# JaneliaSciComp/BigStitcher-Spark

Measured on AMD Instinct MI355X. Metric: tile-pairs/sec phase-correlated (512^3 uint16), higher is better.
Workload: dtype f32+i64; 1 GPU; BASELINE.json configs[1]: 64x512^3 uint16 tile-pairs per GPU, ~10% x-overlap content, ds=1,1,1, peaks=5, subpixel, 8 distinct scenes, no collectives; pairs_per_gpu=64, tile=512^3, parallelism=dp1 hash-sharded pairs

## Files before the change

bigstitcher_spark_amd/csrc/bigstitch.hip:

```cpp

#include "../../include/bigstitch.h"

#include <hip/hip_runtime.h>

#include "rtest_walk.h"
#include "xfft_r4.h"

#include <chrono>
#include <climits>
#include <cmath>
#include <cstdio>
#include <cstdlib>
#include <cstring>
#include <condition_variable>
#include <functional>
#include <map>
#include <mutex>
#include <thread>
#include <string>
#include <vector>
#include <algorithm>

#define LPB_X 4
#define TPL_X 64
#define LPB_S 8
#define TPL_S 64

typedef unsigned long long u64;

struct f2 { float x, y; };

__device__ __forceinline__ f2 cmul(f2 a, f2 b) {
  return {a.x * b.x - a.y * b.y, a.x * b.y + a.y * b.x};
}
__device__ __forceinline__ f2 conjmul(f2 a, f2 b) {
  return {a.x * b.x + a.y * b.y, a.x * b.y - a.y * b.x};
}
__device__ __forceinline__ unsigned brev_n(unsigned j, int log2n) {
  return __brev(j) >> (32 - log2n);
}

template <int ES, int TPL>
__device__ __forceinline__ void fft_lds(f2 *data, long base, int n,
                                        int log2n, int tl, const f2 *tw,
                                        int dir) {
#define D_(e) data[base + (long)(e) * ES]
  int h = 1;
  if (log2n & 1) {
    for (int bf = tl; bf < (n >> 1); bf += TPL) {
      f2 u = D_(2 * bf), v = D_(2 * bf + 1);
      D_(2 * bf) = {u.x + v.x, u.y + v.y};
      D_(2 * bf + 1) = {u.x - v.x, u.y - v.y};
    }
    h = 2;
    __syncthreads();
  }
  for (; h < n; h <<= 2) {
    const int q = n >> 2;
    const int s1 = n / (2 * h), s2 = n / (4 * h);
    for (int g = tl; g < q; g += TPL) {
      int off = g % h, blk = g / h;
      int i = blk * 4 * h + off;
      f2 a = D_(i), b = D_(i + h), c = D_(i + 2 * h), d = D_(i + 3 * h);
      f2 w1 = tw[off * s1];
      if (dir < 0) w1.y = -w1.y;
      f2 t1 = cmul(b, w1), t2 = cmul(d, w1);
      f2 A = {a.x + t1.x, a.y + t1.y}, B = {a.x - t1.x, a.y - t1.y};
      f2 Cc = {c.x + t2.x, c.y + t2.y}, Dd = {c.x - t2.x, c.y - t2.y};
      f2 w2a = tw[off * s2], w2b = tw[(off + h) * s2];
      if (dir < 0) {
        w2a.y = -w2a.y;
        w2b.y = -w2b.y;
      }
      f2 u1 = cmul(Cc, w2a), u2 = cmul(Dd, w2b);
      D_(i) = {A.x + u1.x, A.y + u1.y};
      D_(i + 2 * h) = {A.x - u1.x, A.y - u1.y};
      D_(i + h) = {B.x + u2.x, B.y + u2.y};
      D_(i + 3 * h) = {B.x - u2.x, B.y - u2.y};
    }
    __syncthreads();
  }
#undef D_
}

template <int ES, int TPL>
__device__ __forceinline__ int fft_stockham(f2 *bufA, f2 *bufB, long base,
                                            int n, unsigned long long
                                                        factors,
                                            int tl, const f2 *tw,
// ... 1103 lines not shown
  for (unsigned lid = blockIdx.x * XW_WPB + wv; lid < nlines;
       lid += gridDim.x * XW_WPB) {
    const int z = (int)(lid / (unsigned)in.my);
    const int y = (int)(lid - (unsigned)z * (unsigned)in.my);
    const unsigned short *src =
        in.ptr + (in.oz + z) * in.sxy + (in.oy + y) * in.sx + in.ox;
    f2 v[E];
    if (((size_t)src & 3) == 0 && in.mx >= 2 * h) {
#pragma unroll
      for (int e = 0; e < E; ++e) {
        const unsigned w = ((const unsigned *)src)[lane + 64 * e];
        v[e] = {(float)(w & 0xFFFF), (float)(w >> 16)};
      }
    } else {
#pragma unroll
      for (int e = 0; e < E; ++e) {
        const int j = lane + 64 * e;
        v[e] = {2 * j < in.mx ? (float)src[2 * j] : 0.0f,
                2 * j + 1 < in.mx ? (float)src[2 * j + 1] : 0.0f};
      }
    }
    xf_wave_fft<E, +1>(v, tws, buf, lane);
    xf_wave_sync();
#pragma unroll
    for (int e = 0; e < E; ++e) buf[lane + 64 * e] = v[e];
    xf_wave_sync();
    f2 *o = out + ((long)z * py + y) * cxp;
#pragma unroll
    for (int e = 0; e < E; ++e) {
      const int k = lane + 64 * e;
      const f2 zm = buf[xf_mirror<E>(k)];
      if (k == 0) {
        f2 x0, xh;
        xf_unpack0(v[0], x0, xh);
        o[0] = x0;
        o[h] = xh;
      } else {
        o[k] = xf_unpack(v[e], zm, twu[e]);
      }
    }
  }
}

template <int E>
__global__ __launch_bounds__(64 * XW_WPB) void k_fft_x_inv_r4(
    const f2 *in, float *out, float *rowmax, long cxp, long nlines,
    const f2 *twg, const int *rows, const int *nrows_dev, int store_pcm,
    int store_rowmax) {
  constexpr int h = 64 * E;
  __shared__ f2 xb[XW_WPB][h];
  const int lane = threadIdx.x & 63;
  const int wv = __builtin_amdgcn_readfirstlane(threadIdx.x >> 6);
  f2 *buf = xb[wv];
  xf_twset<E, f2> tws;
  xf_load_tw<E>(tws, twg, lane, -1);
  f2 twp[E];
#pragma unroll
  for (int e = 0; e < E; ++e) twp[e] = twg[lane + 64 * e];
  if (rows) nlines = *nrows_dev;
  for (long li = (long)blockIdx.x * XW_WPB + wv; li < nlines;
       li += (long)gridDim.x * XW_WPB) {
    const long lid = rows ? (long)rows[li] : li;
    const f2 *src = in + lid * cxp;
    f2 v[E];
#pragma unroll
    for (int e = 0; e < E; ++e) {
      const int k = lane + 64 * e;
      v[e] = xf_prep(src[k], src[h - k], twp[e]);
    }
    xf_wave_fft<E, -1>(v, tws, buf, lane);
    if (store_pcm) {
      f2 *o = (f2 *)(out + lid * 2 * h);
#pragma unroll
      for (int e = 0; e < E; ++e)
        o[e * 64 + lane] = v[e];
    }
    if (store_rowmax) {
      float m = fmaxf(v[0].x, v[0].y);
#pragma unroll
      for (int e = 1; e < E; ++e) m = fmaxf(m, fmaxf(v[e].x, v[e].y));
      m = wave_max_f32(m);
      if (lane == 0) rowmax[lid] = m;
    }
  }
}


struct bs_peak {
  float v;
  int pad;
  long long idx;
};

__device__ __forceinline__ bool pk_better(float v, long long i, float v2,
                                          long long i2) {
  return (v > v2) || (v == v2 && i < i2);
}

__device__ void pk_insert(float (&tv)[5], long long (&ti)[5], float v,
                          long long i) {
  if (!pk_better(v, i, tv[4], ti[4])) return;
  tv[4] = v; ti[4] = i;
  for (int k = 4; k > 0 && pk_better(tv[k], ti[k], tv[k - 1], ti[k - 1]);
       --k) {
    float fv = tv[k]; tv[k] = tv[k - 1]; tv[k - 1] = fv;
    long long fi = ti[k]; ti[k] = ti[k - 1]; ti[k - 1] = fi;
  }
}

__device__ void pk_merge_shfl(float (&tv)[5], long long (&ti)[5]) {
  for (int off = 32; off >= 1; off >>= 1) {
    float ov[5]; long long oi[5];
    for (int k = 0; k < 5; ++k) {
      ov[k] = __shfl_down(tv[k], off);
      oi[k] = __shfl_down(ti[k], off);
    }
    for (int k = 0; k < 5; ++k) pk_insert(tv, ti, ov[k], oi[k]);
  }
}

struct pk_raw {
  float4 r[3];
  float el[3], er[3];
};

struct pk_win {
  float4 nm[3];
  float4 raw1;
  float4 cm1;
};

__device__ __forceinline__ pk_win pk_compute(const pk_raw &p, int lane,
                                             int nlt) {
  pk_win o;
#pragma unroll
  for (int k = 0; k < 3; ++k) {
    const float4 r = p.r[k];
    float lw = __shfl_up(r.w, 1);
    float rw = __shfl_down(r.x, 1);
    if (lane == 0) lw = p.el[k];
    if (lane == nlt - 1) rw = p.er[k];
    o.nm[k].x = fmaxf(fmaxf(lw, r.x), r.y);
    o.nm[k].y = fmaxf(fmaxf(r.x, r.y), r.z);
    o.nm[k].z = fmaxf(fmaxf(r.y, r.z), r.w);
    o.nm[k].w = fmaxf(fmaxf(r.z, r.w), rw);
    if (k == 1) {
      o.raw1 = r;
      o.cm1 = {fmaxf(lw, r.y), fmaxf(r.x, r.z), fmaxf(r.y, r.w),
               fmaxf(r.z, rw)};
    }
  }
  return o;
}

__device__ __forceinline__ float4 f4max(float4 a, float4 b) {
  return {fmaxf(a.x, b.x), fmaxf(a.y, b.y), fmaxf(a.z, b.z),
          fmaxf(a.w, b.w)};
}

#define PKW_CZ 64

template <bool UNUSED>
__device__ __forceinline__ void pk_body(const float *pcm, int px, int py,
                                        int pz, bs_peak *wgbuf) {
  __shared__ float wvs[4][5];
  __shared__ long long wis[4][5];
// ... 949 lines not shown
      std::lock_guard<std::mutex> lk(mu);
      stop = true;
    }
    cv.notify_all();
    for (auto &t : th) t.join();
  }
};

struct bs_slot {
  hipStream_t stream = nullptr;
  hipEvent_t peaks_ready = nullptr, done = nullptr;
  f2 *spec = nullptr;
  size_t spec_cap = 0;
  float *pcm = nullptr;
  size_t pcm_cap = 0;
  unsigned short *regbuf[2] = {nullptr, nullptr};
  size_t reg_cap[2] = {0, 0};
  bs_peak *wgpk = nullptr;
  size_t wgpk_cap = 0;
  bs_peak *dmerge = nullptr;
  bs_peak *dtop5 = nullptr;
  float *rowmax = nullptr;
  size_t rowmax_cap = 0;
  int *rowstamp = nullptr;
  size_t rowstamp_cap = 0;
  int *rowlist = nullptr;
  int row_epoch = 0;
  int pcm_sparse = 0;
  int row_listed = 0;
  f2 *twx = nullptr;
  int xinv_r4 = 0;
  int pk_prefilter = 0;
  bs_cand *dcands = nullptr;
  u64 *dsums = nullptr;
  long long *dpkidx = nullptr;
  float *dsubpix = nullptr;
  bs_peak *htop5 = nullptr;
  u64 *hsums = nullptr;
  float *hsubpix = nullptr;
  int Px = 0, Py = 0, Pz = 0, Cx = 0;
  long Cxp = 0;
  bs_region reg[2];
  int m[2][3];
  int dsf[3];
  std::vector<bs_hostcand> hc;
  long long pkidx_h[8];
  int npk = 0;
  size_t out_idx = 0;
  int stage = 0;
};

#define BS_NSLOTS 4

struct bs_ctx {
  int dev;
  int nslots = 2;
  std::map<int, f2 *> twiddles_full;
  hipStream_t stream;
  hipStream_t copy_stream = nullptr;
  bs_pool cpool;
  std::string err;
  std::map<int32_t, bs_view_rec> views;
  std::map<int, f2 *> twiddles;
  bs_slot slot[BS_NSLOTS];
  unsigned long long *synth_acc = nullptr;
  size_t synth_cap = 0;
  void *fuse_out = nullptr;
  size_t fuse_cap = 0;
  bs_dev_view *dviews = nullptr;
  size_t dviews_cap = 0;
  int *dvidx = nullptr;
  size_t dvidx_cap = 0;
  float *dblobs = nullptr;
  size_t dblobs_cap = 0;
  void *hstage[2] = {nullptr, nullptr};
  void *dvol_arena = nullptr;
  size_t dvol_cap = 0;
  hipEvent_t stage_ev[2] = {nullptr, nullptr};
  int peak_full = 0;
  int pcm_rows = 1;
  bs_slot *dbg_slot = nullptr;
  int corr_wide = 1;
  int xfft_fwd_r4 = 1, xfft_inv_r4 = 1;
  float *dbg_pcm = nullptr;
  bs_peak dbg_top5[5] = {};
  long dbg_px = 0, dbg_py = 0, dbg_pz = 0;
  float *dog_box = nullptr, *dog_g1 = nullptr, *dog_g2 = nullptr,
        *dog_d = nullptr;
  size_t dog_box_cap = 0, dog_g1_cap = 0, dog_g2_cap = 0, dog_d_cap = 0;
  long long *dog_cand = nullptr;
  size_t dog_cand_cap = 0;
  struct bs_dog_pt *dog_pts = nullptr;
  size_t dog_pts_cap = 0;
  unsigned int *dog_cnt = nullptr;
  size_t dog_cnt_cap = 0;
  size_t dog_init_cap = 65536;
  void *ip_buf[12] = {};
  size_t ip_cap[12] = {};
  int ip_split = 0;
  void *int_buf[8] = {};
  size_t int_cap[8] = {};
  bs_batch_stats stats{};
  std::vector<bs_ev> evs;
  std::vector<std::pair<hipEvent_t, hipEvent_t>> evpool;
  size_t evused = 0;
  std::mutex mu;
};

#define CHK(ctx, call)                                                      \
  do {                                                                      \
    hipError_t e_ = (call);                                                 \
    if (e_ != hipSuccess) {                                                 \
      (ctx)->err = std::string(#call) + ": " + hipGetErrorString(e_);       \
      return BS_EHIP;                                                       \
    }                                                                       \
  } while (0)

static thread_local std::string g_err;

extern "C" const char *bs_last_error(const bs_ctx *ctx) {
  return ctx ? ctx->err.c_str() : g_err.c_str();
}

static size_t rtest_alloc_bytes(size_t bytes) {
  return (bytes + 15) & ~(size_t)15;
}

static int ensure_dev(bs_ctx *c, void **p, size_t *cap, size_t need) {
  if (need <= *cap) return BS_OK;
  if (*p) (void)hipFree(*p);
  *p = nullptr;
  *cap = 0;
  hipError_t e = hipMalloc(p, need);
  if (e != hipSuccess) {
    c->err = std::string("hipMalloc: ") + hipGetErrorString(e);
    return BS_ENOMEM;
  }
  *cap = need;
  return BS_OK;
}

extern "C" int bs_ctx_create(bs_ctx **out, int device_id) {
  if (!out) return BS_EINVAL;
  int n = 0;
  if (hipGetDeviceCount(&n) != hipSuccess || device_id >= n) {
    g_err = "no HIP device (libbigstitch requires a GPU; the product path "
            "has no CPU fallback)";
    return BS_ENODEV;
  }
  bs_ctx *c = new bs_ctx();
  c->dev = device_id;
  if (const char *e = getenv("BS_SLOTS")) {
    int v = atoi(e);
    if (v >= 1 && v <= BS_NSLOTS) c->nslots = v;
  }
  if (const char *e = getenv("BS_PEAK_MODE"))
    c->peak_full = strcmp(e, "full") == 0;
  if (const char *e = getenv("BS_PCM_MODE"))
    c->pcm_rows = strcmp(e, "full") != 0;
  if (c->peak_full) c->pcm_rows = 0;
  if (const char *e = getenv("BS_CORR_MODE"))
    c->corr_wide = strcmp(e, "legacy") != 0;
  if (const char *e = getenv("BS_XFFT_MODE")) {
    c->xfft_fwd_r4 = strcmp(e, "r4") == 0 || strcmp(e, "r4fwd") == 0;
    c->xfft_inv_r4 = strcmp(e, "r4") == 0 || strcmp(e, "r4inv") == 0;
  }
  if (const char *e = getenv("BS_DOG_INIT_CAP")) {
    long v = atol(e);
    if (v >= 1) c->dog_init_cap = (size_t)v;
  }
  if (const char *e = getenv("BS_IP_SPLIT")) {
    int v = atoi(e);
    if (v >= 1) c->ip_split = v;
  }
  if (hipSetDevice(device_id) != hipSuccess ||
      hipStreamCreate(&c->stream) != hipSuccess ||
      hipStreamCreate(&c->copy_stream) != hipSuccess) {
    delete c;
    g_err = "hip init failed";
    return BS_ENODEV;
  }
  (void)hipFuncSetAttribute((const void *)k_fft_pass,
                            hipFuncAttributeMaxDynamicSharedMemorySize,
                            160 * 1024);
  (void)hipFuncSetAttribute((const void *)k_fft_pass_m,
                            hipFuncAttributeMaxDynamicSharedMemorySize,
                            160 * 1024);
  (void)hipFuncSetAttribute((const void *)k_fft_x_fwd_m,
                            hipFuncAttributeMaxDynamicSharedMemorySize,
                            160 * 1024);
  (void)hipFuncSetAttribute((const void *)k_fft_x_inv_m,
                            hipFuncAttributeMaxDynamicSharedMemorySize,
                            160 * 1024);
  (void)hipFuncSetAttribute((const void *)k_fft_pass_glds<2>,
                            hipFuncAttributeMaxDynamicSharedMemorySize,
                            160 * 1024);
  (void)hipFuncSetAttribute((const void *)k_fft_pass_glds<4>,
                            hipFuncAttributeMaxDynamicSharedMemorySize,
                            160 * 1024);
  (void)hipFuncSetAttribute((const void *)k_fft_pass_glds<8>,
                            hipFuncAttributeMaxDynamicSharedMemorySize,
                            160 * 1024);
  (void)hipFuncSetAttribute((const void *)k_fft_z_fused<1>,
                            hipFuncAttributeMaxDynamicSharedMemorySize,
                            160 * 1024);
  (void)hipFuncSetAttribute((const void *)k_fft_z_fused<2>,
                            hipFuncAttributeMaxDynamicSharedMemorySize,
                            160 * 1024);
  (void)hipFuncSetAttribute((const void *)k_fft_z_fused<4>,
                            hipFuncAttributeMaxDynamicSharedMemorySize,
                            160 * 1024);
  (void)hipFuncSetAttribute((const void *)k_fft_z_fused<8>,
                            hipFuncAttributeMaxDynamicSharedMemorySize,
                            160 * 1024);
  (void)hipFuncSetAttribute((const void *)k_fft_x_fwd,
                            hipFuncAttributeMaxDynamicSharedMemorySize,
                            64 * 1024);
  (void)hipFuncSetAttribute((const void *)k_fft_x_inv,
                            hipFuncAttributeMaxDynamicSharedMemorySize,
                            64 * 1024);
  bool ok = true;
  for (int s = 0; s < BS_NSLOTS; ++s) {
    bs_slot &sl = c->slot[s];
    ok = ok && hipStreamCreate(&sl.stream) == hipSuccess &&
         hipEventCreateWithFlags(&sl.peaks_ready, hipEventDisableTiming) ==
             hipSuccess &&
         hipEventCreateWithFlags(&sl.done, hipEventDisableTiming) ==
             hipSuccess &&
         hipMalloc(&sl.dmerge, 64 * 5 * sizeof(bs_peak)) == hipSuccess &&
         hipMalloc(&sl.dtop5, 6 * sizeof(bs_peak)) == hipSuccess &&
         hipMalloc(&sl.rowlist, (2 + 9 * BS_PEAK_ROWS_CAP) * sizeof(int)) ==
             hipSuccess &&
         hipMalloc(&sl.dcands, 64 * sizeof(bs_cand)) == hipSuccess &&
         hipMalloc(&sl.dsums, 64 * 5 * sizeof(u64)) == hipSuccess &&
         hipMalloc(&sl.dpkidx, 8 * sizeof(long long)) == hipSuccess &&
         hipMalloc(&sl.dsubpix, 8 * 7 * sizeof(float)) == hipSuccess &&
         hipHostMalloc(&sl.htop5, 6 * sizeof(bs_peak)) == hipSuccess &&
         hipHostMalloc(&sl.hsums, 64 * 5 * sizeof(u64)) == hipSuccess &&
         hipHostMalloc(&sl.hsubpix, 8 * 7 * sizeof(float)) == hipSuccess;
  }
  if (!ok) {
    delete c;
    g_err = "alloc failed";
    return BS_ENOMEM;
  }
  *out = c;
  return BS_OK;
}
// ... 490 lines not shown
  CHK(c, hipEventSynchronize(sl->peaks_ready));
  return BS_OK;
}


static int stitch_phaseA(bs_ctx *c, bs_slot *sl, const bs_pair_desc &pd,
                         const bs_stitch_params *prm, size_t out_idx) {
  auto ita = c->views.find(pd.view_a);
  auto itb = c->views.find(pd.view_b);
  if (ita == c->views.end() || itb == c->views.end()) {
    c->err = "view not uploaded";
    return BS_ENOVIEW;
  }
  int *ds = sl->dsf;
  ds[0] = prm->ds[0] > 0 ? prm->ds[0] : 1;
  ds[1] = prm->ds[1] > 0 ? prm->ds[1] : 1;
  ds[2] = prm->ds[2] > 0 ? prm->ds[2] : 1;
  bool dsall1 = ds[0] == 1 && ds[1] == 1 && ds[2] == 1;
  for (int t = 0; t < 2; ++t) {
    const bs_view_rec &vr = t == 0 ? ita->second : itb->second;
    const int64_t *off = t == 0 ? pd.off_a : pd.off_b;
    const int64_t *size = t == 0 ? pd.size_a : pd.size_b;
    for (int d = 0; d < 3; ++d) {
      if (off[d] < 0 || size[d] <= 0 || off[d] + size[d] > vr.dims[d]) {
        c->err = "pair interval out of view bounds";
        return BS_EINVAL;
      }
      sl->m[t][d] = (int)(size[d] / ds[d]);
      if (sl->m[t][d] < 1) {
        c->err = "pair interval smaller than downsampling factor";
        return BS_EINVAL;
      }
    }
    if (dsall1) {
      sl->reg[t] = {vr.dptr, vr.dims[0], vr.dims[0] * vr.dims[1],
                    off[0], off[1], off[2],
                    sl->m[t][0], sl->m[t][1], sl->m[t][2]};
    } else {
      size_t need = rtest_alloc_bytes((size_t)sl->m[t][0] * sl->m[t][1] *
                                      sl->m[t][2] * 2);
      int rc = ensure_dev(c, (void **)&sl->regbuf[t], &sl->reg_cap[t], need);
      if (rc) return rc;
      bs_region src = {vr.dptr, vr.dims[0], vr.dims[0] * vr.dims[1],
                       off[0], off[1], off[2], 0, 0, 0};
      long nrows = (long)sl->m[t][1] * sl->m[t][2];
      bs_tim tt(c, BS_K_DOWNSAMPLE, sl->stream);
      hipLaunchKernelGGL(k_downsample, dim3(std::min(4096L, nrows)),
                         dim3(256), 0, sl->stream, src, sl->regbuf[t],
                         sl->m[t][0], sl->m[t][1], sl->m[t][2], ds[0], ds[1],
                         ds[2]);
      sl->reg[t] = {sl->regbuf[t], sl->m[t][0],
                    (long)sl->m[t][0] * sl->m[t][1], 0, 0, 0,
                    sl->m[t][0], sl->m[t][1], sl->m[t][2]};
    }
  }
  const bool fastpad = prm->pad_mode == 1;
  auto pad1 = [&](int m01) {
    return fastpad ? next_fast_even(std::max(m01, 8))
                   : next_pow2(m01);
  };
  int Px = pad1(std::max(sl->m[0][0], sl->m[1][0]));
  int Py = pad1(std::max(sl->m[0][1], sl->m[1][1]));
  int Pz = pad1(std::max(sl->m[0][2], sl->m[1][2]));
  if (Px > 1024 || Py > 1024 || Pz > 1024 || Px < 8) {
    c->err = "FFT size unsupported (need 8..1024 per axis)";
    return BS_EUNSUP;
  }
  int Cx = Px / 2 + 1;
  long Cxp = (Cx + 15) & ~15L;
  sl->Px = Px; sl->Py = Py; sl->Pz = Pz; sl->Cx = Cx; sl->Cxp = Cxp;
  sl->out_idx = out_idx;
  size_t spec_half = (size_t)Pz * Py * Cxp;
  int rc = ensure_dev(c, (void **)&sl->spec, &sl->spec_cap,
                      2 * spec_half * sizeof(f2));
  if (rc) return rc;
  size_t pcm_n = (size_t)Pz * Py * Px;
  rc = ensure_dev(c, (void **)&sl->pcm, &sl->pcm_cap, pcm_n * sizeof(float));
  if (rc) return rc;
  rc = peak_ensure(c, sl);
  if (rc) return rc;
  f2 *twx = is_pow2(Px) ? get_twiddle(c, Px) : get_twiddle_full(c, Px);
  f2 *twy = is_pow2(Py) ? get_twiddle(c, Py) : get_twiddle_full(c, Py);
  f2 *twz = is_pow2(Pz) ? get_twiddle(c, Pz) : get_twiddle_full(c, Pz);
  if (!twx || !twy || !twz) {
    c->err = "twiddle alloc failed";
    return BS_ENOMEM;
  }
  f2 *spec[2] = {sl->spec, sl->spec + spec_half};
  for (int t = 0; t < 2; ++t) {
    long nlines = (long)sl->reg[t].my * sl->reg[t].mz;
    bs_tim tt(c, BS_K_FFT_X_FWD, sl->stream);
    if (!is_pow2(Px)) {
      long ngrp = (nlines + LPB_X - 1) / LPB_X;
      size_t lds = ((Px / 2) + 2 * (size_t)LPB_X * (Px / 2)) * sizeof(f2);
      hipLaunchKernelGGL(k_fft_x_fwd_m, dim3(std::min(4096L, ngrp)),
                         dim3(LPB_X * TPL_X), lds, sl->stream, sl->reg[t],
                         spec[t], Px, bs_factorize(Px / 2), Cxp, Py, twx);
    } else if (Px >= 128 && Px <= 1024) {
      long ngrp = (nlines + XW_WPB - 1) / XW_WPB;
      dim3 g(std::min(4096L, ngrp)), b(64 * XW_WPB);
      if (Px == 128)
        hipLaunchKernelGGL(k_fft_x_fwd_w<1>, g, b, 0, sl->stream,
                           sl->reg[t], spec[t], Cxp, Py, twx);
      else if (Px == 256)
        hipLaunchKernelGGL(k_fft_x_fwd_w<2>, g, b, 0, sl->stream,
                           sl->reg[t], spec[t], Cxp, Py, twx);
      else if (Px == 512 && c->xfft_fwd_r4)
        hipLaunchKernelGGL(k_fft_x_fwd_r4<4>, g, b, 0, sl->stream,
                           sl->reg[t], spec[t], Cxp, Py, twx);
      else if (Px == 512)
        hipLaunchKernelGGL(k_fft_x_fwd_w<4>, g, b, 0, sl->stream,
                           sl->reg[t], spec[t], Cxp, Py, twx);
      else if (c->xfft_fwd_r4)
        hipLaunchKernelGGL(k_fft_x_fwd_r4<8>, g, b, 0, sl->stream,
                           sl->reg[t], spec[t], Cxp, Py, twx);
      else
        hipLaunchKernelGGL(k_fft_x_fwd_w<8>, g, b, 0, sl->stream,
                           sl->reg[t], spec[t], Cxp, Py, twx);
    } else {
      long ngrp = (nlines + LPB_X - 1) / LPB_X;
      size_t lds = ((Px / 4) + (size_t)LPB_X * (Px / 2)) * sizeof(f2);
      hipLaunchKernelGGL(k_fft_x_fwd, dim3(std::min(4096L, ngrp)),
                         dim3(LPB_X * TPL_X), lds, sl->stream, sl->reg[t],
                         spec[t], Px, ilog2(Px), Cx, Cxp, Py, twx);
    }
  }
  int nchunks = (Cx + LPB_S - 1) / LPB_S;
  static const bool yglds = getenv("BS_Y_GLDS") != nullptr;
  auto launch_y = [&](f2 *sp, int ngroups, int valid, int dir) {
    if (!is_pow2(Py)) {
      size_t lds = (Py + 2 * (size_t)LPB_S * Py) * sizeof(f2);
      hipLaunchKernelGGL(k_fft_pass_m,
                         dim3(std::min(4096L, (long)ngroups * nchunks)),
                         dim3(LPB_S * TPL_S), lds, sl->stream, sp,
                         (const f2 *)nullptr, sp, Py, bs_factorize(Py),
                         Cxp, (long)Py * Cxp, Cx, nchunks, ngroups, valid,
                         dir, 1.0f, twy);
    } else if (yglds && Py >= 256) {
      size_t lds2 = ((Py / 2) + 2 * (size_t)LPB_S * Py) * sizeof(f2);
      long nwg = (long)ngroups * nchunks;
      dim3 g(std::min(512L, nwg)), b(LPB_S * TPL_S);
      if (Py == 256)
        hipLaunchKernelGGL(k_fft_pass_glds<2>, g, b, lds2, sl->stream, sp,
                           Py, ilog2(Py), Cxp, (long)Py * Cxp, Cx, nchunks,
                           ngroups, valid, dir, twy);
      else if (Py == 512)
        hipLaunchKernelGGL(k_fft_pass_glds<4>, g, b, lds2, sl->stream, sp,
                           Py, ilog2(Py), Cxp, (long)Py * Cxp, Cx, nchunks,
                           ngroups, valid, dir, twy);
      else
        hipLaunchKernelGGL(k_fft_pass_glds<8>, g, b, lds2, sl->stream, sp,
                           Py, ilog2(Py), Cxp, (long)Py * Cxp, Cx, nchunks,
                           ngroups, valid, dir, twy);
    } else {
      size_t lds = ((Py / 2) + (size_t)LPB_S * Py) * sizeof(f2);
      hipLaunchKernelGGL(k_fft_pass,
                         dim3(std::min(4096L, (long)ngroups * nchunks)),
                         dim3(LPB_S * TPL_S), lds, sl->stream, sp,
                         (const f2 *)nullptr, sp, Py, ilog2(Py), Cxp,
                         (long)Py * Cxp, Cx, nchunks, ngroups, valid, dir,
                         1.0f, twy);
    }
  };
  for (int t = 0; t < 2; ++t) {
    bs_tim tt(c, BS_K_FFT_Y_FWD, sl->stream);
    launch_y(spec[t], sl->reg[t].mz, sl->reg[t].my, +1);
  }
  if (!is_pow2(Pz)) {
    float scale = 1.0f / ((float)Px * (float)Py * (float)Pz);
    size_t lds = (Pz + 2 * (size_t)LPB_S * Pz) * sizeof(f2);
    dim3 g(std::min(4096L, (long)Py * nchunks)), b(LPB_S * TPL_S);
    for (int t = 0; t < 2; ++t) {
      bs_tim tt(c, BS_K_FFT_Z_FWD, sl->stream);
      hipLaunchKernelGGL(k_fft_pass_m, g, b, lds, sl->stream, spec[t],
                         (const f2 *)nullptr, spec[t], Pz,
                         bs_factorize(Pz), (long)Py * Cxp, Cxp, Cx,
                         nchunks, Py, sl->reg[t].mz, +1, 1.0f, twz);
    }
    bs_tim tt(c, BS_K_FFT_Z_INV, sl->stream);
    hipLaunchKernelGGL(k_fft_pass_m, g, b, lds, sl->stream, spec[0],
                       spec[1], spec[0], Pz, bs_factorize(Pz),
                       (long)Py * Cxp, Cxp, Cx, nchunks, Py, Pz, -1,
                       scale, twz);
  } else {
    float scale = 1.0f / ((float)Px * (float)Py * (float)Pz);
    size_t lds = ((Pz / 2) + (size_t)LPB_S * Pz) * sizeof(f2);
    bs_tim tt(c, BS_K_FFT_Z_INV, sl->stream);
    dim3 g(std::min(4096L, (long)Py * nchunks)), b(LPB_S * TPL_S);
    auto zf = [&](auto kern) {
      hipLaunchKernelGGL(kern, g, b, lds, sl->stream, spec[0], spec[1],
                         Pz, ilog2(Pz), (long)Py * Cxp, Cxp, Cx, nchunks,
                         Py, sl->reg[0].mz, sl->reg[1].mz, scale, twz);
    };
    static const bool z_r8 = getenv("BS_Z_R8") != nullptr;
    static const bool z_nt = getenv("BS_Z_NT") != nullptr;
    if (Pz <= 128)
      zf(k_fft_z_fused<1>);
    else if (Pz == 256)
      zf(k_fft_z_fused<2>);
    else if (Pz == 512)
      z_r8 ? zf(k_fft_z_fused_r8<4>)
           : z_nt ? zf(k_fft_z_fused_nt<4>) : zf(k_fft_z_fused_np<4>);
    else
      z_r8 ? zf(k_fft_z_fused_r8<8>)
           : z_nt ? zf(k_fft_z_fused_nt<8>) : zf(k_fft_z_fused_np<8>);
  }
  {
    size_t lds = ((Py / 2) + (size_t)LPB_S * Py) * sizeof(f2);
    bs_tim tt(c, BS_K_FFT_Y_INV, sl->stream);
    (void)lds;
    launch_y(spec[0], Pz, Py, -1);
  }
  sl->twx = twx;
  sl->xinv_r4 = c->xfft_inv_r4;
  sl->pcm_sparse = c->pcm_rows && !c->peak_full;
  sl->row_listed = sl->pcm_sparse;
  {
    bs_tim tt(c, BS_K_FFT_X_INV, sl->stream);
    launch_x_inv(sl, sl->pcm_sparse ? X_INV_MAX : X_INV_FULL);
  }
  c->dbg_pcm = sl->pcm;
  c->dbg_slot = sl;
  c->dbg_px = Px;
  c->dbg_py = Py;
  c->dbg_pz = Pz;
  rc = peak_issue(c, sl, c->peak_full != 0);
  if (rc) return rc;
  sl->stage = 1;
  return BS_OK;
}

static bool cand_box(const int ma[3], const int mb[3], const int s[3],
                     bs_hostcand *h) {
  int lo[3], hi[3];
  for (int d = 0; d < 3; ++d) {
    lo[d] = std::max(0, -s[d]);
    hi[d] = std::min(ma[d], mb[d] - s[d]);
    if (hi[d] <= lo[d]) return false;
  }
  h->gc = {lo[0], lo[1], lo[2], hi[0] - lo[0], hi[1] - lo[1],
           hi[2] - lo[2], s[0], s[1], s[2]};
  h->n = (long)(hi[0] - lo[0]) * (hi[1] - lo[1]) * (hi[2] - lo[2]);
  return true;
}

static int rtest_issue(bs_ctx *c, bs_slot *sl) {
  std::stable_sort(sl->hc.begin(), sl->hc.end(),
                   [](const bs_hostcand &x, const bs_hostcand &y) {
                     return x.gc.sz < y.gc.sz;
                   });
  std::vector<bs_cand> gc(sl->hc.size());
  for (size_t i = 0; i < sl->hc.size(); ++i) gc[i] = sl->hc[i].gc;
  CHK(c, hipMemcpyAsync(sl->dcands, gc.data(), gc.size() * sizeof(bs_cand),
                        hipMemcpyHostToDevice, sl->stream));
  CHK(c, hipMemsetAsync(sl->dsums, 0, gc.size() * 5 * sizeof(u64),
                        sl->stream));
  CHK(c, hipStreamSynchronize(sl->stream));
  {
    int maxz = 1;
    for (auto &h : sl->hc)
      maxz = std::max(maxz, h.gc.loz + h.gc.nz);
    bs_tim tt(c, BS_K_CORR, sl->stream);
    static const int corr_gy = [] {
      const char *e = getenv("BS_CORR_GY");
      return e ? atoi(e) : 8;
    }();
    hipLaunchKernelGGL(c->corr_wide ? k_rtest_wide : k_rtest,
                       dim3((unsigned)maxz, corr_gy), dim3(256),
                       0, sl->stream, sl->reg[0], sl->reg[1], sl->dcands,
                       (int)gc.size(), sl->dsums);
  }
  CHK(c, hipMemcpyAsync(sl->hsums, sl->dsums,
                        sl->hc.size() * 5 * sizeof(u64),
                        hipMemcpyDeviceToHost, sl->stream));
  return BS_OK;
}

static int stitch_phaseB(bs_ctx *c, bs_slot *sl,
                         const bs_stitch_params *prm) {
// ... 1516 lines not shown
```

Measured before the change: 387.6 tile-pairs/s.

## Add register-resident radix-8 FFT kernels for 512-point Y and fused Z passes

Adds new strided FFT kernels for 512-point lines built as three radix-8 stages held in registers. Each workgroup handles pairs of adjacent complex lines loaded as float4, with swizzled LDS exchanges between stages and twiddles cached in LDS. Both the Y pass and the fused Z forward/cross-power/inverse pass switch to these kernels by default when the size is 512. The aim is fewer LDS round trips and barriers than the radix-2 shared-memory passes, at the cost of higher register pressure and more complex indexing.

```diff
diff --git a/bigstitcher_spark_amd/csrc/bigstitch.hip b/bigstitcher_spark_amd/csrc/bigstitch.hip
--- a/bigstitcher_spark_amd/csrc/bigstitch.hip
+++ b/bigstitcher_spark_amd/csrc/bigstitch.hip
@@ -5,6 +5,7 @@
 
 #include "rtest_walk.h"
 #include "xfft_r4.h"
+#include "sfft_r8.h"
 
 #include <chrono>
 #include <climits>
@@ -1274,6 +1275,187 @@
       m = wave_max_f32(m);
       if (lane == 0) rowmax[lid] = m;
     }
+  }
+}
+
+
+__device__ __forceinline__ void sf_load(sf_lines<f2> &v, const f2 *src,
+                                        long base2, long estride, int lane,
+                                        int valid, int nl, bool full) {
+  const f2 *row0 = src + base2;
+  const f2 *p = row0 + lane * estride;
+  if (full) {
+#pragma unroll
+    for (int r = 0; r < 8; ++r, p += 64 * estride) {
+      const bool in = lane + 64 * r < valid;
+      float4 q = *(const float4 *)(in ? p : row0);
+      if (!in) q = {0.0f, 0.0f, 0.0f, 0.0f};
+      sf_split(q, v.a[r], v.b[r]);
+    }
+    return;
+  }
+#pragma unroll
+  for (int r = 0; r < 8; ++r, p += 64 * estride) {
+    float4 q = {0.0f, 0.0f, 0.0f, 0.0f};
+    if (lane + 64 * r < valid) {
+      if (nl == 2) {
+        q = *(const float4 *)p;
+      } else if (nl == 1) {
+        const f2 t = *p;
+        q.x = t.x;
+        q.y = t.y;
+      }
+    }
+    sf_split(q, v.a[r], v.b[r]);
+  }
+}
+
+__device__ __forceinline__ void sf_store(const sf_lines<f2> &v, f2 *dst,
+                                         long base2, long estride, int lane,
+                                         int nl, bool full) {
+  f2 *p = dst + base2 + lane * estride;
+#pragma unroll
+  for (int s = 0; s < 8; ++s, p += 64 * estride) {
+    if (full || nl == 2)
+      *(float4 *)p = sf_join<float4>(v.a[s], v.b[s]);
+    else if (nl == 1)
+      *p = v.a[s];
+  }
+}
+
+__device__ __forceinline__ int sf_fresh(int x) {
+  asm volatile("" : "+v"(x));
+  return x;
+}
+
+struct sf_ids {
+  int tid, ow;
+  __device__ __forceinline__ int pl() const { return sf_io_pair(sf_fresh(tid)); }
+  __device__ __forceinline__ int il() const { return sf_io_lane(sf_fresh(tid)); }
+  __device__ __forceinline__ int ol() const { return sf_own_lane(sf_fresh(tid)); }
+};
+
+__device__ __forceinline__ void sf_x_io_to_own(sf_lines<f2> &v, float4 *tile,
+                                               const sf_ids &id) {
+  sf_put<float4, 1>(tile, sf_put_base(id.pl(), id.il(), 1), v);
+  __syncthreads();
+  sf_get<float4>(tile, sf_get_base(id.ow, id.ol()), v);
+}
+
+__device__ __forceinline__ void sf_x_own_to_io(sf_lines<f2> &v, float4 *tile,
+                                               const sf_ids &id) {
+  xf_wave_sync();
+  sf_put<float4, 8>(tile, sf_put_base(id.ow, id.ol(), 8), v);
+  __syncthreads();
+  sf_get<float4>(tile, sf_get_base(id.pl(), id.il()), v);
+}
+
+template <int L>
+__device__ __forceinline__ void sf_x_own(sf_lines<f2> &v, float4 *tile,
+                                         const sf_ids &id) {
+  xf_wave_sync();
+  sf_put<float4, L>(tile, sf_put_base(id.ow, id.ol(), L), v);
+  xf_wave_sync();
+  sf_get<float4>(tile, sf_get_base(id.ow, id.ol()), v);
+}
+
+__device__ __forceinline__ void sf_fill_tw(f2 *twt, const f2 *tw2n, int tid) {
+  for (int i = tid; i < SF_TWN; i += SF_THREADS)
+    twt[i] = sf_tw_entry(tw2n, i);
+  __syncthreads();
+}
+
+template <int DIR>
+__device__ __forceinline__ void sf_stage_tw(sf_lines<f2> &v, const f2 *twt,
+                                            int si, int lane) {
+  f2 w[7];
+  sf_get_tw(twt, si, lane, w);
+  sf_stage<DIR>(v, w);
+}
+
+struct sf_tile_pos {
+  long base2;
+  int nl;
+  bool full;
+};
+
+__device__ __forceinline__ sf_tile_pos sf_locate(long wg, int nchunks,
+                                                 long gstride, int nlines,
+                                                 int pl) {
+  const int group = (int)(wg / nchunks);
+  const int x0 = (int)(wg % nchunks) * (2 * SF_PAIRS);
+  const int x2 = x0 + 2 * pl;
+  return {(long)group * gstride + x2, min(max(nlines - x2, 0), 2),
+          x0 + 2 * SF_PAIRS <= nlines};
+}
+
+template <int DIR>
+__global__ __launch_bounds__(SF_THREADS)
+__attribute__((amdgpu_waves_per_eu(4))) void k_fft_pass_r8(
+    f2 *data, long estride, long gstride, int nlines, int nchunks,
+    int ngroups, int valid, const f2 *tw2n) {
+  __shared__ float4 tile[SF_TILE];
+  __shared__ f2 twt[SF_TWN];
+  const sf_ids id = {(int)threadIdx.x,
+                     __builtin_amdgcn_readfirstlane(
+                         sf_own_pair((int)threadIdx.x))};
+  sf_fill_tw(twt, tw2n, id.tid);
+  const long nwg = (long)ngroups * nchunks;
+  for (long wg = blockIdx.x; wg < nwg; wg += gridDim.x) {
+    const sf_tile_pos tp = sf_locate(wg, nchunks, gstride, nlines, id.pl());
+    sf_lines<f2> v;
+    sf_load(v, data, tp.base2, estride, id.il(), valid, tp.nl, tp.full);
+    sf_stage0<DIR>(v);
+    sf_x_io_to_own(v, tile, id);
+    sf_stage_tw<DIR>(v, twt, 1, id.ol());
+    sf_x_own_to_io(v, tile, id);
+    sf_stage_tw<DIR>(v, twt, 2, id.il());
+    sf_store(v, data, tp.base2, estride, id.il(), tp.nl, tp.full);
+    __syncthreads();
+  }
+}
+
+__device__ __forceinline__ void sf_fwd_to_owner(sf_lines<f2> &v, float4 *tile,
+                                                const f2 *twt,
+                                                const sf_ids &id) {
+  sf_stage0<+1>(v);
+  sf_x_io_to_own(v, tile, id);
+  sf_stage_tw<+1>(v, twt, 1, id.ol());
+  sf_x_own<8>(v, tile, id);
+  sf_stage_tw<+1>(v, twt, 2, id.ol());
+}
+
+__global__ __launch_bounds__(SF_THREADS)
+__attribute__((amdgpu_waves_per_eu(3))) void k_fft_z_fused_r8x(
+    f2 *a, const f2 *b, long estride, long gstride, int nlines, int nchunks,
+    int ngroups, int valid_a, int valid_b, float scale, const f2 *tw2n) {
+  __shared__ float4 tile[SF_TILE];
+  __shared__ f2 twt[SF_TWN];
+  const sf_ids id = {(int)threadIdx.x,
+                     __builtin_amdgcn_readfirstlane(
+                         sf_own_pair((int)threadIdx.x))};
+  sf_fill_tw(twt, tw2n, id.tid);
+  const long nwg = (long)ngroups * nchunks;
+  for (long wg = blockIdx.x; wg < nwg; wg += gridDim.x) {
+    const sf_tile_pos tp = sf_locate(wg, nchunks, gstride, nlines, id.pl());
+    sf_lines<f2> va, vb;
+    sf_load(va, a, tp.base2, estride, id.il(), valid_a, tp.nl, tp.full);
+    sf_load(vb, b, tp.base2, estride, id.il(), valid_b, tp.nl, tp.full);
+    sf_fwd_to_owner(va, tile, twt, id);
+    __syncthreads();
+    sf_fwd_to_owner(vb, tile, twt, id);
+#pragma unroll
+    for (int r = 0; r < 8; ++r) {
+      va.a[r] = sf_crosspower(va.a[r], vb.a[r], scale);
+      va.b[r] = sf_crosspower(va.b[r], vb.b[r], scale);
+    }
+    sf_stage0<-1>(va);
+    sf_x_own<1>(va, tile, id);
+    sf_stage_tw<-1>(va, twt, 1, id.ol());
+    sf_x_own_to_io(va, tile, id);
+    sf_stage_tw<-1>(va, twt, 2, id.il());
+    sf_store(va, a, tp.base2, estride, id.il(), tp.nl, tp.full);
+    __syncthreads();
   }
 }
 
@@ -2389,6 +2571,7 @@
   bs_slot *dbg_slot = nullptr;
   int corr_wide = 1;
   int xfft_fwd_r4 = 1, xfft_inv_r4 = 1;
+  int sfft_y_r8 = 1, sfft_z_r8 = 1;
   float *dbg_pcm = nullptr;
   bs_peak dbg_top5[5] = {};
   long dbg_px = 0, dbg_py = 0, dbg_pz = 0;
@@ -2471,6 +2654,10 @@
   if (const char *e = getenv("BS_XFFT_MODE")) {
     c->xfft_fwd_r4 = strcmp(e, "r4") == 0 || strcmp(e, "r4fwd") == 0;
     c->xfft_inv_r4 = strcmp(e, "r4") == 0 || strcmp(e, "r4inv") == 0;
+  }
+  if (const char *e = getenv("BS_SFFT_MODE")) {
+    c->sfft_y_r8 = strcmp(e, "r8") == 0 || strcmp(e, "r8y") == 0;
+    c->sfft_z_r8 = strcmp(e, "r8") == 0 || strcmp(e, "r8z") == 0;
   }
   if (const char *e = getenv("BS_DOG_INIT_CAP")) {
     long v = atol(e);
@@ -3127,7 +3314,10 @@
   f2 *twx = is_pow2(Px) ? get_twiddle(c, Px) : get_twiddle_full(c, Px);
   f2 *twy = is_pow2(Py) ? get_twiddle(c, Py) : get_twiddle_full(c, Py);
   f2 *twz = is_pow2(Pz) ? get_twiddle(c, Pz) : get_twiddle_full(c, Pz);
-  if (!twx || !twy || !twz) {
+  f2 *tws = (Py == SF_N && c->sfft_y_r8) || (Pz == SF_N && c->sfft_z_r8)
+                ? get_twiddle(c, 2 * SF_N)
+                : twy;
+  if (!twx || !twy || !twz || !tws) {
     c->err = "twiddle alloc failed";
     return BS_ENOMEM;
   }
@@ -3181,6 +3371,14 @@
                          (const f2 *)nullptr, sp, Py, bs_factorize(Py),
                          Cxp, (long)Py * Cxp, Cx, nchunks, ngroups, valid,
                          dir, 1.0f, twy);
+    } else if (Py == SF_N && c->sfft_y_r8 && !yglds) {
+      dim3 g(std::min(4096L, (long)ngroups * nchunks)), b(SF_THREADS);
+      if (dir > 0)
+        hipLaunchKernelGGL(k_fft_pass_r8<+1>, g, b, 0, sl->stream, sp, Cxp,
+                           (long)Py * Cxp, Cx, nchunks, ngroups, valid, tws);
+      else
+        hipLaunchKernelGGL(k_fft_pass_r8<-1>, g, b, 0, sl->stream, sp, Cxp,
+                           (long)Py * Cxp, Cx, nchunks, ngroups, valid, tws);
     } else if (yglds && Py >= 256) {
       size_t lds2 = ((Py / 2) + 2 * (size_t)LPB_S * Py) * sizeof(f2);
       long nwg = (long)ngroups * nchunks;
@@ -3239,7 +3437,12 @@
     };
     static const bool z_r8 = getenv("BS_Z_R8") != nullptr;
     static const bool z_nt = getenv("BS_Z_NT") != nullptr;
-    if (Pz <= 128)
+    if (Pz == SF_N && c->sfft_z_r8 && !z_r8 && !z_nt)
+      hipLaunchKernelGGL(k_fft_z_fused_r8x, g, dim3(SF_THREADS), 0,
+                         sl->stream, spec[0], (const f2 *)spec[1],
+                         (long)Py * Cxp, Cxp, Cx, nchunks, Py, sl->reg[0].mz,
+                         sl->reg[1].mz, scale, tws);
+    else if (Pz <= 128)
       zf(k_fft_z_fused<1>);
     else if (Pz == 256)
       zf(k_fft_z_fused<2>);
diff --git a/bigstitcher_spark_amd/csrc/sfft_r8.h b/bigstitcher_spark_amd/csrc/sfft_r8.h
--- /dev/null
+++ b/bigstitcher_spark_amd/csrc/sfft_r8.h
@@ -0,0 +1,121 @@
+#ifndef BS_SFFT_R8_H
+#define BS_SFFT_R8_H
+
+#include <math.h>
+
+#include "xfft_r4.h"
+
+#define SF_N 512
+#define SF_PAIRS 4
+#define SF_THREADS 256
+#define SF_TILE (SF_PAIRS * SF_N)
+
+BS_XF_FN int sf_io_pair(int tid) { return tid & (SF_PAIRS - 1); }
+BS_XF_FN int sf_io_lane(int tid) { return tid >> 2; }
+BS_XF_FN int sf_own_pair(int tid) { return tid >> 6; }
+BS_XF_FN int sf_own_lane(int tid) { return tid & 63; }
+
+BS_XF_FN int sf_twist(int p) { return (2 * p) ^ (9 * (p >> 1)); }
+
+BS_XF_FN int sf_idx(int p, int m) {
+  return SF_N * p + (xf_swz<8>(m) ^ sf_twist(p));
+}
+
+template <class C>
+struct sf_lines {
+  C a[8], b[8];
+};
+
+template <class C, class Q>
+BS_XF_FN void sf_split(const Q &q, C &a, C &b) {
+  a = {q.x, q.y};
+  b = {q.z, q.w};
+}
+
+template <class Q, class C>
+BS_XF_FN Q sf_join(C a, C b) {
+  return {a.x, a.y, b.x, b.y};
+}
+
+template <int DIR, class C>
+BS_XF_FN C sf_twmul(C a, C b) {
+  return DIR > 0 ? C{a.x * b.x - a.y * b.y, a.x * b.y + a.y * b.x}
+                 : C{a.x * b.x + a.y * b.y, a.y * b.x - a.x * b.y};
+}
+
+template <int DIR, class C>
+BS_XF_FN void sf_stage0(sf_lines<C> &v) {
+  xf_bfly<DIR>(v.a);
+  xf_bfly<DIR>(v.b);
+}
+
+template <int DIR, class C>
+BS_XF_FN void sf_stage(sf_lines<C> &v, const C (&w)[7]) {
+  BS_XF_UNROLL
+  for (int r = 1; r < 8; ++r) v.a[r] = sf_twmul<DIR>(v.a[r], w[r - 1]);
+  xf_bfly<DIR>(v.a);
+  BS_XF_UNROLL
+  for (int r = 1; r < 8; ++r) v.b[r] = sf_twmul<DIR>(v.b[r], w[r - 1]);
+  xf_bfly<DIR>(v.b);
+}
+
+BS_XF_FN int sf_put_base(int p, int lane, int L) {
+  return sf_idx(p, xf_dst<8>(L, lane, 0));
+}
+BS_XF_FN int sf_put_xor(int L, int s) { return L == 1 ? s : 9 * s; }
+BS_XF_FN int sf_get_base(int p, int lane) { return sf_idx(p, lane); }
+BS_XF_FN int sf_get_xor(int r) { return (64 * r) | (8 * (r & 1)); }
+
+template <class Q, int L, class T, class C>
+BS_XF_FN void sf_put(T tile, int base, const sf_lines<C> &v) {
+  static_assert(L == 1 || L == 8, "the two exchanges of three stages");
+  BS_XF_UNROLL
+  for (int s = 0; s < 8; ++s)
+    tile[base ^ sf_put_xor(L, s)] = sf_join<Q>(v.a[s], v.b[s]);
+}
+
+template <class Q, class T, class C>
+BS_XF_FN void sf_get(T tile, int base, sf_lines<C> &v) {
+  BS_XF_UNROLL
+  for (int r = 0; r < 8; ++r) {
+    const Q q = tile[base ^ sf_get_xor(r)];
+    sf_split(q, v.a[r], v.b[r]);
+  }
+}
+
+#define SF_TW1 (7 * 8)
+#define SF_TWN (SF_TW1 + 7 * 64)
+
+BS_XF_FN int sf_tw_slot(int si, int r, int lane) {
+  return si == 1 ? (r - 1) * 8 + (lane & 7) : SF_TW1 + (r - 1) * 64 + lane;
+}
+
+template <class C>
+BS_XF_FN C sf_tw_entry(const C *twn, int i) {
+  const int si = i < SF_TW1 ? 1 : 2;
+  const int k = i < SF_TW1 ? i : i - SF_TW1;
+  const int r = (si == 1 ? k >> 3 : k >> 6) + 1;
+  const int lane = si == 1 ? k & 7 : k & 63;
+  return xf_tw<8>(twn, xf_tw_q<8>(xf_L<8>(si), lane, r), +1);
+}
+
+template <class C, class T>
+BS_XF_FN void sf_get_tw(T tab, int si, int lane, C (&w)[7]) {
+  BS_XF_UNROLL
+  for (int r = 1; r < 8; ++r) w[r - 1] = tab[sf_tw_slot(si, r, lane)];
+}
+
+template <class C>
+BS_XF_FN C sf_crosspower(C a, C b, float scale) {
+  const C q = {a.x * b.x + a.y * b.y, a.x * b.y - a.y * b.x};
+  const float m = q.x * q.x + q.y * q.y;
+  C v = {0.0f, 0.0f};
+  if (m > 1e-40f) {
+    const float s = scale / sqrtf(m);
+    v.x = q.x * s;
+    v.y = q.y * s;
+  }
+  return v;
+}
+
+#endif
```

Result: faster. 429.0 tile-pairs/s (median of 6 runs) (+10.7%).
